# pletzer/nemoflux

Hardware: AMD Instinct MI355X
Metric: edge-flux integrals/sec (higher is better)
Workload: dtype f64; 1 GPU; C4 ORCA12-like 3600x1800x75x12 in total (strong: 900 (t,z) slabs cut 1 way), psi=(1+10*z)*(t+1)*arctan2(y, x+180)/(2*pi), README singular transect + 64 node-snapped transects; nx=3600, ny=1800, nz=75, nt_global=12, target_segments=2229, weight_entries=15468144, parallelism=(t,z)-slab sharding x1, 1 all-reduce, resident_outputs=integratedVelocity [4][ncell] + |eU|,|eV| every step

## Files before the change

nemoflux_amd/csrc/nf_capi_field.hip:

```cpp
#include "nf_capi.h"

using namespace nf;

static int g_batch_steps = 1;
static long g_batch_cellsteps = 32l << 20;
static int g_partial_full = 0;
static int g_use_graph = 1;
static int g_inner_signed = 1;
static int g_k3_pairs = 1;
static int g_inner_interleaved = -1;
static int g_class_window = 32;
static int g_joint_window = 32;
static int g_joint_skip = 1;
static long g_knob_version = 0;

namespace nf {
int field_tuning_set(const char *name, int value)
{
    ++g_knob_version;
    if (!strcmp(name, "batch_steps")) {
        g_batch_steps = value;
        return NF_OK;
    }
    if (!strcmp(name, "batch_cellsteps_m")) {
        if (!(value >= 0 && value <= 2047)) return -1;
        g_batch_cellsteps = (long)value << 20;
        return NF_OK;
    }
    if (!strcmp(name, "partial_step_planes")) {
        g_partial_full = value != 0;
        return NF_OK;
    }
    if (!strcmp(name, "graph")) {
        g_use_graph = value != 0;
        return NF_OK;
    }
    if (!strcmp(name, "pass_inner_signed")) {
        g_inner_signed = value != 0;
        return NF_OK;
    }
    if (!strcmp(name, "pass_k3_pairs")) {
        g_k3_pairs = value != 0;
        return NF_OK;
    }
    if (!strcmp(name, "pass_inner_interleaved")) {
        if (!(value >= -1 && value <= 1)) return -1;
        g_inner_interleaved = value;
        return NF_OK;
    }
    if (!strcmp(name, "class_window")) {
        if (!(value >= 1 && value <= kClassWindowMax)) return -1;
        g_class_window = value;
        return NF_OK;
    }
    if (!strcmp(name, "joint_window")) {
        if (!(value >= 1 && value <= kClassWindowMax)) return -1;
        g_joint_window = value;
        return NF_OK;
    }
    if (!strcmp(name, "joint_skip")) {
        if (!(value == 0 || value == 1)) return -1;
        g_joint_skip = value;
        return NF_OK;
    }
    if (!strcmp(name, "area_chunk")) return area_chunk_set(value);
    if (!strcmp(name, "gross_chunk")) return gross_chunk_set(value);
    if (!strcmp(name, "crossing_chunk")) return crossing_chunk_set(value);
    return -1;
}
}

struct Series {
    const void *p[2] = {nullptr, nullptr};
    long nt = 0;
    int dtype = NF_F64, on_device = 1;
    double fill = std::numeric_limits<double>::quiet_NaN();
    double fill2 = std::numeric_limits<double>::quiet_NaN();
    DevArray<char> stage[2];
};

// ... 352 lines not shown
               std::string(what) + ": this form does not take per-cell thicknesses yet and a cell thickness is set; "
                                   "nf_field_set_cell_thickness(NULL) clears it");
    return NF_OK;
}

static FluxArgs flux_args(const StepInput &in)
{
    return FluxArgs{in.u, in.v, in.dtype, in.ncell, in.ny, in.nx, in.z0, in.z1, in.thickness, in.arcE, in.arcN, in.fill,
                    in.fill2, in.scale, in.sverdrup};
}

static int field_integral(nf_field *f, const double *planes, double *scratch, double *rows, int nsteps = 1,
                          long data_stride = 0, long row_stride = 0)
{
    const Transects tr = field_transects(f);
    return launch_integral(f->ws, planes, f->ncell, 2, f->nx, tr.tr_offsets_dev, tr.ntransect, scratch, rows, f->stream, nsteps,
                           data_stride, row_stride);
}

template <typename Step>
static int field_sync(nf_field *f, size_t n, double *host, Step step)
{
    NF_TRY(f->row.reserve(n > 0 ? n : 1));
    NF_TRY(step(f->row.get()));
    if (host && n > 0) NF_HIP(hipMemcpyAsync(host, f->row.get(), sizeof(double) * n, hipMemcpyDeviceToHost, f->stream));
    NF_HIP(hipStreamSynchronize(f->stream));
    return NF_OK;
}

struct StepForm {
    bool inner = false;
    double *pair_buf = nullptr;
    bool interleaved = false;
};

static int field_step_async(nf_field *f, long t, double *row_dev, StepForm form = {})
{
    const int rowlen = field_row_length(f);
    const bool reduce = row_dev && rowlen > 0 && !form.pair_buf;
    NF_TRY(field_ready(f, "compute", reduce));
    NF_REQUIRE(t >= 0 && t < f->uv.nt, NF_ERR_ARG, "compute: time index out of range");
    const Levels lv = field_levels(f, t);
    if (lv.z1 <= lv.z0) {
        if (row_dev && rowlen > 0) NF_HIP(hipMemsetAsync(row_dev, 0, sizeof(double) * rowlen, f->stream));
        return NF_OK;
    }
    StepInput in;
    NF_TRY(field_step_input(f, t, lv, &in));
    CellThick ct;
    NF_TRY(field_cell_thick(f, t, lv, &ct));
    FluxArgs a = flux_args(in);
    a.iV = f->geo.iV.get();
    if (form.pair_buf) a.iV = form.interleaved ? form.pair_buf : form.pair_buf - f->ncell;
    a.absU = f->geo.abs.get();
    a.absV = f->geo.abs.get() + f->ncell;
    a.maxbits = f->geo.maxbits.get();
    const bool partial = (lv.z0 > 0 || lv.z1 < (int)f->nz) && !g_partial_full;
    a.signed_only = (f->compact || partial || form.inner) && (ct.e3u || flux_supports_signed_only(a));
    NF_REQUIRE(!form.pair_buf || a.signed_only, NF_ERR_STATE, "compute: a step into a pair buffer must be signed-only");
    NF_REQUIRE(!form.interleaved || (form.pair_buf && !ct.e3u && !partial && flux_supports_interleaved(a)), NF_ERR_STATE,
               "compute: the interleaved form is a whole step of a pair on K1's two-field kernel");
    a.interleaved = form.interleaved;
    if (!form.pair_buf) f->derived_stale = a.signed_only != 0;
    NF_TRY(field_launch_flux(f, a, ct.e3u ? &ct : nullptr));
    if (reduce) {
        NF_TRY(field_integral(f, f->geo.iV.get(), f->scratch.get(), row_dev));
        NF_TRY(field_timed_k3_end(f));
    }
    return NF_OK;
}

static int field_raw_step_begin(nf_field *f, const char *what, long t, int tracer, double *rows_dev, size_t nrows, Levels *lv)
{
    const std::string w(what);
    NF_REQUIRE(t >= 0 && t < f->uv.nt, NF_ERR_ARG, w + ": time index out of range");
    if (tracer) NF_TRY(field_matches_uv(f, f->tau.dtype, f->tau.nt, w, "tracer"));
    if (tracer == 2 && f->sig.p[0])
        NF_TRY(field_matches_uv(f, f->sig.dtype, f->sig.nt, w, "class tracer"));
    const size_t rowlen = field_row_length(f);
    *lv = rowlen > 0 ? field_levels(f, t) : Levels{};
    if (rowlen > 0 && lv->z1 <= lv->z0) NF_HIP(hipMemsetAsync(rows_dev, 0, sizeof(double) * rowlen * nrows, f->stream));
    return NF_OK;
}

static int field_tracer_input(nf_field *f, Series &s, long t, Levels lv, TracerIn *in)
{
    NF_TRY(field_stage(f, s, 0, t, lv, &in->tau));
    in->fill = s.fill;
    in->fill2 = s.fill2;
    in->ref = &s == &f->tau ? f->tau_ref : 0.0;
    in->wrap_x = f->tau_wrap;
    return NF_OK;
}

static int field_profile_async(nf_field *f, long t, double *prof_dev, bool tracer = false)
// ... 297 lines not shown
    a.edges = f->class_edges.dev.get();
    a.nedges = nedges;
    a.window = window;
    a.tr = field_transects(f);
    a.scratch = f->class_scratch.get();
    a.scratch_len = f->class_scratch.size();
    a.rows = rows_dev;
    a.nz = (int)f->nz;
    return launch_gross_class_remap(a, f->stream);
}

static int field_class_area_async(nf_field *f, long t, double *rows_dev)
{
    const int nedges = (int)f->class_edges.host.size();
    const size_t nrows = 2 * ((size_t)nedges + 2);
    Levels lv;
    NF_TRY(field_raw_step_begin(f, "compute_class_area", t, 2, rows_dev, nrows, &lv));
    if (lv.z1 <= lv.z0) return NF_OK;
    NF_TRY(f->class_edges.upload((size_t)kMaxClassEdges, f->stream));
    ClassAreaArgs a;
    NF_TRY(field_joint_buffers(f, "compute_class_area", kClassAreaEntryBytes, lv, nrows, &a));
    NF_TRY(field_step_input(f, t, lv, &a.in));
    NF_TRY(field_tracer_input(f, f->tau, t, lv, &a.carry));
    a.cls = a.carry;
    if (f->sig.p[0]) NF_TRY(field_tracer_input(f, f->sig, t, lv, &a.cls));
    NF_TRY(field_cell_thick(f, t, lv, &a.th));
    a.edges = f->class_edges.dev.get();
    a.nedges = nedges;
    a.tr = field_transects(f);
    a.rows = rows_dev;
    return launch_class_area(a, f->stream);
}

static int field_pair_async(nf_field *f, long t, double *rows_dev, bool last, bool last_pair, bool interleaved)
{
    const int rowlen = field_row_length(f);
    StepForm first, second;
    first.inner = true;
    first.pair_buf = f->geo.pair[0].get();
    first.interleaved = interleaved;
    second.inner = g_inner_signed && !last;
    if (interleaved && second.inner && !last_pair) {
        second.pair_buf = f->geo.pair[1].get();
        second.interleaved = true;
    }
    NF_TRY(field_step_async(f, t, nullptr, first));
    NF_TRY(field_step_async(f, t + 1, nullptr, second));
    const double *uvB = second.pair_buf ? second.pair_buf : f->geo.iV.get() + f->ncell;
    NF_TRY(launch_integral_pair(field_transects(f), first.pair_buf, uvB, f->ncell, f->nx, f->scratch.get(),
                                rows_dev + (size_t)t * rowlen, rowlen, f->stream, first.interleaved, second.interleaved));
    NF_TRY(field_timed_k3_end(f));
    return NF_OK;
}

static long batch_cell_steps() { return g_batch_cellsteps; }

static bool field_can_batch(const nf_field *f)
{
    return g_batch_steps && !f->e3.p[0] && f->uv.on_device && f->uv.nt >= 2 && f->uv.nt < 65536 &&
           f->uv.nt * f->ncell <= batch_cell_steps() && f->ncell <= (1l << 20) && f->weights_built;
}

static bool field_pass_pairs(const nf_field *f)
{
    if (!g_k3_pairs || integral_uses_edges() || !f->geo.pair[0].get() || !f->weights_built) return false;
    const size_t step_bytes = (size_t)f->nz * f->ncell * elem_size(f->uv.dtype);
    FluxArgs a{};
    a.u = f->uv.on_device ? f->uv.p[0] : nullptr;
    a.v = f->uv.on_device ? f->uv.p[1] : nullptr;
    a.dtype = f->uv.dtype;
    a.ncell = f->ncell;
    return flux_supports_signed_only(a) && (!f->uv.on_device || step_bytes % 16 == 0);
}

static bool field_pass_interleaved(const nf_field *f)
{
    const bool on = g_inner_interleaved < 0 ? f->uv.dtype == NF_F64 : g_inner_interleaved != 0;
    if (!on || f->compact || f->e3.p[0]) return false;
    FluxArgs a{};
    a.u = f->uv.on_device ? f->uv.p[0] : nullptr;
    a.v = f->uv.on_device ? f->uv.p[1] : nullptr;
    a.dtype = f->uv.dtype;
    a.ncell = f->ncell;
    return flux_supports_interleaved(a);
}

static int field_prepare_pass(nf_field *f)
{
    if (!g_k3_pairs || integral_uses_edges() || !f->geo.iV.get()) return NF_OK;
    const PassSteps p = field_pass_steps(f);
    if (p.wb - p.wa < 2) return NF_OK;
    if (!f->geo.pair[0].get()) NF_TRY(f->geo.pair[0].alloc((size_t)f->ncell * 2));
    if (!f->geo.pair[1].get() && p.wb - p.wa >= 4 && field_pass_interleaved(f)) NF_TRY(f->geo.pair[1].alloc((size_t)f->ncell * 2));
    return NF_OK;
}

static int field_zero_unowned_rows(nf_field *f, double *rows_dev)
{
    const int rowlen = field_row_length(f);
    const PassSteps p = field_pass_steps(f);
    if (rowlen <= 0) return NF_OK;
    if (p.ta > 0) NF_HIP(hipMemsetAsync(rows_dev, 0, sizeof(double) * rowlen * (size_t)p.ta, f->stream));
    if (p.tb < f->uv.nt)
        NF_HIP(hipMemsetAsync(rows_dev + (size_t)p.tb * rowlen, 0, sizeof(double) * rowlen * (size_t)(f->uv.nt - p.tb),
                              f->stream));
    return NF_OK;
}

static int field_all_steps_direct(nf_field *f, double *rows_dev, bool zero_rows = true)
{
    const int rowlen = field_row_length(f);
    const PassSteps p = field_pass_steps(f);
    if (zero_rows) NF_TRY(field_zero_unowned_rows(f, rows_dev));
    const bool pairs = field_pass_pairs(f) && rowlen > 0;
    const long pa = pairs ? p.wa + (p.wb - p.wa) % 2 : p.wb;
    const bool interleaved = pairs && field_pass_interleaved(f) && (p.wb - pa < 4 || f->geo.pair[1].get());
    for (long t = p.ta; t < p.tb;) {
        const bool last = t + 1 == p.tb;
        if (t >= pa && t + 1 < p.wb) {
            NF_TRY(field_pair_async(f, t, rows_dev, t + 2 == p.tb, t + 2 == p.wb, interleaved));
            t += 2;
        } else {
            StepForm form;
            form.inner = g_inner_signed && !last;
            NF_TRY(field_step_async(f, t, rows_dev + (size_t)t * rowlen, form));
            t += 1;
        }
    }
    return NF_OK;
}

static int field_all_steps_batched(nf_field *f, double *rows_dev)
{
    const int rowlen = field_row_length(f);
    const size_t n = (size_t)f->ncell;
    nf_field::Geometry &g = f->geo;
    if (g.batch_steps != f->uv.nt) {
        NF_TRY(g.iVb.alloc(n * 4 * f->uv.nt));
        NF_TRY(g.absb.alloc(n * 2 * f->uv.nt));
        NF_TRY(g.zr.alloc((size_t)2 * f->uv.nt));
        NF_HIP(hipMemsetAsync(g.iVb.get(), 0, sizeof(double) * n * 4 * f->uv.nt, f->stream));
        g.batch_steps = f->uv.nt;
        g.batch_version = -1;
    }
    if (g.batch_version != f->version) {
        NF_TRY(g.scratchb.alloc((size_t)std::max(f->ws.nrec, f->ws.nent) * f->uv.nt));
        std::vector<int> zr((size_t)2 * f->uv.nt);
        for (long t = 0; t < f->uv.nt; ++t) {
            const Levels lv = field_levels(f, t);
            zr[2 * t] = lv.z0;
            zr[2 * t + 1] = lv.z1;
        }
        NF_HIP(hipMemcpy(g.zr.get(), zr.data(), sizeof(int) * zr.size(), hipMemcpyHostToDevice));
// ... 227 lines not shown
    for (size_t p = 0; p < f->polylines.size(); ++p) {
        polyline_segments(f->polylines[p].data(), (int)(f->polylines[p].size() / 3), f->poly_cc[p], segs, cc);
        f->tr_off.push_back((int)cc.size());
    }
    f->weights_built = false;
    f->prof_scratch.reset();
    f->tprof_scratch.reset();
    f->area_scratch.reset();
    f->gross_scratch.reset();
    f->crossings.reset();
    f->class_scratch.reset();
    f->joint_table.reset();
    f->joint_flags.reset();
    f->joint_scratch.reset();
    const int bw = build_weights(f->geo.xy.get(), f->ncell, segs.data(), cc.data(), (int)cc.size(), periodX, &f->ws, f->stream,
                                 f->skip_unsupported, f->overlap_warn, nullptr, f->nx);
    if (bw != NF_OK) {
        for (size_t q = 0; q < f->ws.coverage.size(); ++q)
            if ((long)q == (long)f->ws.over_seg) {
                size_t p = 0;
                while (p + 2 < f->tr_off.size() && (size_t)f->tr_off[p + 1] <= q) ++p;
                char buf[320];
                snprintf(buf, sizeof buf,
                         "nf_field_build_weights: transect %zu, target segment %zu is covered %.9g times by the cells of the "
                         "grid: cells overlap along it (a cell wrapped across the date line with periodX = 0, or duplicated "
                         "/ folded cells that are not identical), so part of the line would be counted twice",
                         p, q - (size_t)f->tr_off[p], f->ws.coverage[q]);
                set_error(buf);
                break;
            }
        return bw;
    }
    if (integral_uses_edges()) NF_TRY(fold_weights(&f->ws, f->ncell, f->nx, f->stream));
    NF_TRY(f->tr_off_dev.alloc(f->tr_off.size()));
    NF_TRY(f->scratch.alloc((size_t)2 * std::max(f->ws.nrec, f->ws.nent)));
    NF_HIP(hipMemcpy(f->tr_off_dev.get(), f->tr_off.data(), sizeof(int) * f->tr_off.size(), hipMemcpyHostToDevice));
    f->weights_built = true;
    ++f->version;
    return NF_OK;
}
NF_API_CATCH

int nf_field_num_transects(nf_field **self, int *n)
try {
    NF_REQUIRE(self && *self && n, NF_ERR_ARG, "nf_field_num_transects: null argument");
    *n = (int)(*self)->polylines.size();
    return NF_OK;
}
NF_API_CATCH
int nf_field_num_segments(nf_field **self, int *nseg_total)
try {
    NF_REQUIRE(self && *self && nseg_total, NF_ERR_ARG, "nf_field_num_segments: null argument");
    NF_REQUIRE((*self)->weights_built, NF_ERR_STATE, "nf_field_num_segments: build_weights first");
    *nseg_total = (*self)->ws.nseg;
    return NF_OK;
}
NF_API_CATCH
int nf_field_segment_offsets(nf_field **self, int *offsets)
try {
    NF_REQUIRE(self && *self && offsets, NF_ERR_ARG, "nf_field_segment_offsets: null argument");
    NF_REQUIRE((*self)->weights_built, NF_ERR_STATE, "nf_field_segment_offsets: build_weights first");
    memcpy(offsets, (*self)->tr_off.data(), sizeof(int) * (*self)->tr_off.size());
    return NF_OK;
}
NF_API_CATCH
int nf_field_num_weights(nf_field **self, size_t *n)
// ... 933 lines not shown
```

nemoflux_amd/csrc/nf_common.h:

```cpp
#pragma once
#include <hip/hip_runtime.h>
#include <cstdint>
#include <cstdio>
#include <string>
#include <cmath>
#include <initializer_list>
#include <mutex>
#include <vector>

#include "../../include/nemoflux_amd.h"

namespace nf {

constexpr int kWave = 64;
constexpr int kBlock = 256;
constexpr int kXcds = 8;
constexpr double kDeg2Rad = 3.14159265358979323846 / 180.0;
constexpr double kEarthRadiusSv = 6371000.0;

void set_error(const std::string &msg);
int hip_fail(hipError_t e, const char *what, const char *file, int line);

#define NF_HIP(call)                                                   \
    do {                                                               \
// ... 78 lines not shown
    double m = 1.0;
    for (double c : {seg4[0], seg4[1], seg4[0] + seg4[2], seg4[1] + seg4[3]}) m = std::fabs(c) > m ? std::fabs(c) : m;
    return (cov - 1.0) * len > kCoverLenTol * m;
}

int launch_geometry(const void *blon, const void *blat, int dtype, long ncell, double *xy, double *arc4,
                    double *arcE, double *arcN, unsigned long long *box_keys, hipStream_t s);
int launch_corner_table_from_points(const double *points, long ncell, double *xy, hipStream_t s);
int launch_points_from_corner_table(const double *xy, long ncell, double *points, hipStream_t s);
double box_key_to_double(unsigned long long k);

struct StepBatch {
    int nsteps = 0;
    long in_stride = 0;
    const int *zr = nullptr;
};

struct FluxArgs {
    const void *u, *v;
    int dtype;
    long ncell, ny, nx;
    int z0, z1;
    const double *thickness;
    const double *arcE, *arcN;
    double fill;
    double fill2 = __builtin_nan("");
    double scale;
    int sverdrup;
    double *iV, *absU, *absV;
    unsigned long long *maxbits;
    StepBatch batch;
    int signed_only = 0;
    int interleaved = 0;
    hipEvent_t mid_event = nullptr;
    bool *mid_recorded = nullptr;
};
int launch_flux(const FluxArgs &a, hipStream_t s);
bool flux_supports_signed_only(const FluxArgs &a);
bool flux_supports_interleaved(const FluxArgs &a);
int launch_expand_planes(double *iV, double *absUV, long ncell, long ny, long nx, hipStream_t s);
int tuning_set(const char *name, int value);
long tuning_version();
int launch_planes_to_aos(const double *planes, long ncell, double *aos, hipStream_t s);

template <typename T>
class DevArray {
public:
    DevArray() = default;
    DevArray(const DevArray &) = delete;
    DevArray &operator=(const DevArray &) = delete;
    DevArray(DevArray &&o) noexcept : p_(o.p_), n_(o.n_) { o.p_ = nullptr, o.n_ = 0; }
    DevArray &operator=(DevArray &&o) noexcept
    {
        if (this != &o) {
            reset();
            p_ = o.p_, n_ = o.n_;
            o.p_ = nullptr, o.n_ = 0;
        }
        return *this;
    }
    ~DevArray() { reset(); }
    int alloc(size_t n)
    {
        reset();
        void *q = nullptr;
        NF_HIP(hipMalloc(&q, n ? sizeof(T) * n : (sizeof(T) > 16 ? sizeof(T) : 16)));
        p_ = static_cast<T *>(q);
        n_ = n ? n : 1;
        return NF_OK;
    }
    int reserve(size_t n, bool *grown = nullptr)
    {
// ... 3 lines not shown
    }
    void reset()
    {
        if (p_) (void)hipFree(p_);
        p_ = nullptr, n_ = 0;
    }
    T *get() const { return p_; }
    size_t size() const { return n_; }

private:
    T *p_ = nullptr;
    size_t n_ = 0;
};

struct WeightSet {
    long nrec = 0;
    DevArray<int> cell;
    DevArray<double> w4;
    DevArray<int> seg;
    DevArray<double> tab;
    int nseg = 0;
    DevArray<int> seg_start;
    std::vector<double> coverage;
    int over_seg = -1;
    long dropped = 0;
    struct EdgeEntry {
        int elem;
        int seg;
        double w;
    };
    long nent = 0;
    DevArray<EdgeEntry> ent;
    DevArray<int> ent_start;
    long entries() const { return 4 * nrec; }
    void release() { *this = WeightSet(); }
};
int fold_weights(WeightSet *ws, long ncell, long nx, hipStream_t s);
int weights_to_host(const WeightSet &ws, int64_t *cell_edge, double *weight, int *seg);
struct Box4;
struct LocatorBoxes {
    std::vector<DevArray<Box4>> level;
    std::vector<long> count;
    const double *xy = nullptr;
    long ncell = 0;
    double period = -1.0;
    std::mutex mtx;
    void release();
};
int build_weights(const double *xy, long ncell, const double *segs_host, const int *seg_cc_host, int nseg,
                  double periodX, WeightSet *out, hipStream_t s, int skip_unsupported = 0, int overlap_warn = 0,
                  LocatorBoxes *boxes = nullptr, long row_length = 0);
void weights_trim_scratch();

struct Transects {
    const WeightSet *ws = nullptr;
    const int *tr_offsets_dev = nullptr;
    int ntransect = 0;
    long row_length() const { return ws->nseg + ntransect; }
};

void integral_use_edges(int on);
int integral_uses_edges();
int launch_integral(const WeightSet &ws, const double *data, long ncell, int planes, long nx,
                    const int *tr_offsets_dev, int ntransect, double *scratch, double *row, hipStream_t s,
                    int nsteps = 1, long data_stride = 0, long row_stride = 0, const int *rec_cells = nullptr);
int launch_integral_pair(const Transects &tr, const double *uvA, const double *uvB, long ncell, long nx, double *scratch,
                         double *row, long row_stride, hipStream_t s, bool a_interleaved = false, bool b_interleaved = false);

struct StepInput {
// ... 299 lines not shown
```

nemoflux_amd/csrc/nf_flux.hip:

```cpp
#include <cstring>

#include "nf_common.h"

namespace nf {

template <typename T, int VEC> struct vec_t;
typedef double dvec2 __attribute__((ext_vector_type(2)));
typedef float fvec4 __attribute__((ext_vector_type(4)));
template <> struct vec_t<double, 2> { using type = dvec2; };
template <> struct vec_t<float, 4> { using type = fvec4; };
template <> struct vec_t<double, 1> { using type = double; };
template <> struct vec_t<float, 1> { using type = float; };

template <typename T, int VEC> struct Lanes {
    T x[VEC];
};

template <typename T, int VEC, bool NT>
__device__ inline Lanes<T, VEC> load_cells(const T *p)
{
    using V = typename vec_t<T, VEC>::type;
    Lanes<T, VEC> r;
    V v = NT ? __builtin_nontemporal_load(reinterpret_cast<const V *>(p)) : *reinterpret_cast<const V *>(p);
    __builtin_memcpy(&r, &v, sizeof(V));
// ... 50 lines not shown
        if (j0 + 1 < ny) store1<NTS>(p0 + c0 + nx, eV[0]);
        store1<NTS>(p3 + ((i0 + 1 < nx) ? c0 + 1 : c0 + 1 - nx), eU[0]);
    } else {
#pragma unroll
        for (int k = 0; k < VEC; k += 2) {
            store2<NTS>(p1 + c0 + k, eU[k], eU[k + 1], true);
            store2<NTS>(p2 + c0 + k, eV[k], eV[k + 1], true);
            store2<NTS>(aU + c0 + k, fabs(eU[k]), fabs(eU[k + 1]), true);
            store2<NTS>(aV + c0 + k, fabs(eV[k]), fabs(eV[k + 1]), true);
        }
        if (i0 + VEC <= nx) {
            if (j0 + 1 < ny) {
                const bool al = (nx & 1u) == 0;
#pragma unroll
                for (int k = 0; k < VEC; k += 2) store2<NTS>(p0 + c0 + nx + k, eV[k], eV[k + 1], al);
            }
#pragma unroll
            for (int k = 0; k < VEC; ++k) store1<NTS>(p3 + ((i0 + k + 1 < nx) ? c0 + k + 1 : c0 + k + 1 - nx), eU[k]);
        } else {
#pragma unroll
            for (int k = 0; k < VEC; ++k) {
                const long c = c0 + k;
                const unsigned j = (unsigned)(c / nx);
                const unsigned i = (unsigned)(c - (long)j * nx);
                if (j + 1 < ny) store1<NTS>(p0 + c + nx, eV[k]);
                store1<NTS>(p3 + ((i + 1 < nx) ? c + 1 : c + 1 - nx), eU[k]);
            }
        }
    }
}

constexpr int kFormSignedOnly = 16;
constexpr int kFormInterleaved = 32;
constexpr int kFormNestedLoads = 128;
constexpr int kFormTwoFills = 256;
#ifdef NF_TUNING_BUILD
constexpr int kDiagNoStores = 1, kDiagNoFix = 2, kDiagNoMax = 4, kDiagNoArc = 8, kDiagPlainStores = 64;
#else
constexpr int kDiagNoStores = 0, kDiagNoFix = 0, kDiagNoMax = 0, kDiagNoArc = 0, kDiagPlainStores = 0;
#endif

template <typename T, int VEC, int UZ, bool NT, int BLOCK, int CH, int FORM = 0>
__global__ __launch_bounds__(BLOCK) void k_flux(const T *__restrict__ u, const T *__restrict__ v, long ncell,
                                                unsigned ny, unsigned nx, int z0, int z1,
                                                const double *__restrict__ thickness,
                                                const double *__restrict__ arcE, const double *__restrict__ arcN,
                                                T fill, double scale, int sverdrup, double *__restrict__ iV,
                                                double *__restrict__ absUV, unsigned long long *maxbits,
                                                unsigned ntiles, int xcd_map, StepBatch sb, T fill2)
{
#ifndef NF_TUNING_BUILD
    static_assert((FORM & ~(kFormSignedOnly | kFormInterleaved | kFormNestedLoads | kFormTwoFills)) == 0, "diagnostic forms exist only in tuning builds");
#endif
    const unsigned tile = xcd_map ? xcd_tile(blockIdx.x, gridDim.x) : blockIdx.x;
    if (sb.zr) {
        const long tb = blockIdx.y;
        u += tb * sb.in_stride;
        v += tb * sb.in_stride;
        iV += tb * 4 * ncell;
        absUV += tb * 2 * ncell;
        z0 = sb.zr[2 * tb];
        z1 = sb.zr[2 * tb + 1];
    }
    double tmax = 0.0;
    if (tile < ntiles) {
        const long base = (long)tile * BLOCK * VEC * CH + (long)threadIdx.x * VEC;
        constexpr long kChunk = (long)BLOCK * VEC;
        bool on[CH];
        double accU[CH][VEC], accV[CH][VEC];
#pragma unroll
        for (int q = 0; q < CH; ++q) {
            on[q] = base + q * kChunk < ncell;
#pragma unroll
            for (int k = 0; k < VEC; ++k) accU[q][k] = accV[q][k] = 0.0;
        }
        const T *pu = u + (long)z0 * ncell + base;
        const T *pv = v + (long)z0 * ncell + base;
        for (int z = z0; z < z1; z += UZ) {
            const int nlev = z1 - z < UZ ? z1 - z : UZ;
            Lanes<T, VEC> lu[UZ][CH], lv[UZ][CH];
            if (CH == 1 && !(FORM & kFormNestedLoads)) {
#pragma unroll
                for (int k = 0; k < 2 * UZ; ++k) {
                    const int r = k / 2;
                    if (r < nlev && on[0]) {
                        if ((k & 1) == 0) lu[r][0] = load_cells<T, VEC, NT>(pu + (long)r * ncell);
                        else lv[r][0] = load_cells<T, VEC, NT>(pv + (long)r * ncell);
                    }
                }
            } else {
#pragma unroll
                for (int r = 0; r < UZ; ++r)
                    if (r < nlev) {
#pragma unroll
                        for (int q = 0; q < CH; ++q)
                            if (on[q]) {
                                lu[r][q] = load_cells<T, VEC, NT>(pu + (long)r * ncell + q * kChunk);
                                lv[r][q] = load_cells<T, VEC, NT>(pv + (long)r * ncell + q * kChunk);
                            }
                    }
            }
#pragma unroll
            for (int r = 0; r < UZ; ++r)
                if (r < nlev) {
                    const double th = thickness[z + r];
#pragma unroll
                    for (int q = 0; q < CH; ++q)
                        if (on[q]) {
#pragma unroll
                            for (int k = 0; k < VEC; ++k) {
                                if (FORM & kFormTwoFills) {
                                    accU[q][k] = fma(th, fixed2<T>(lu[r][q].x[k], fill, fill2), accU[q][k]);
                                    accV[q][k] = fma(th, fixed2<T>(lv[r][q].x[k], fill, fill2), accV[q][k]);
                                } else {
                                    accU[q][k] = fma(th, (FORM & kDiagNoFix) ? (double)lu[r][q].x[k] : fixed<T>(lu[r][q].x[k], fill), accU[q][k]);
                                    accV[q][k] = fma(th, (FORM & kDiagNoFix) ? (double)lv[r][q].x[k] : fixed<T>(lv[r][q].x[k], fill), accV[q][k]);
                                }
                            }
                        }
                }
            pu += (long)UZ * ncell;
            pv += (long)UZ * ncell;
        }
#pragma unroll
        for (int q = 0; q < CH; ++q)
            if (on[q]) {
                const long c0 = base + q * kChunk;
                double eU[VEC], eV[VEC];
#pragma unroll
                for (int k = 0; k < VEC; ++k) {
                    eU[k] = +accU[q][k] * ((FORM & kDiagNoArc) ? 1.5 : arcE[c0 + k]);
                    eV[k] = -accV[q][k] * ((FORM & kDiagNoArc) ? 1.5 : arcN[c0 + k]);
                    if (sverdrup) {
                        eU[k] *= scale;
                        eV[k] *= scale;
                    }
                    tmax = fmax(tmax, fmax(fabs(eU[k]), fabs(eV[k])));
                }
                if (FORM & kFormInterleaved) {
#pragma unroll
                    for (int k = 0; k < VEC; ++k) store2<true>(iV + 2 * (c0 + k), eU[k], eV[k], true);
                } else if (FORM & kFormSignedOnly) {
#pragma unroll
                    for (int k = 0; k < VEC; k += 2) {
                        store2<true>(iV + ncell + c0 + k, eU[k], eU[k + 1], true);
                        store2<true>(iV + 2 * ncell + c0 + k, eV[k], eV[k + 1], true);
                    }
                } else if (!(FORM & kDiagNoStores)) store_cells<VEC, !(FORM & kDiagPlainStores)>(c0, eU, eV, ncell, ny, nx, iV, absUV);
            }
    }
    for (int o = 32; o > 0; o >>= 1) tmax = fmax(tmax, __shfl_xor(tmax, o, kWave));
    if ((threadIdx.x & (kWave - 1)) == 0 && tmax > 0.0 && !(FORM & kDiagNoMax)) {
        unsigned long long b;
        __builtin_memcpy(&b, &tmax, 8);
        if (b > __hip_atomic_load(maxbits, __ATOMIC_RELAXED, __HIP_MEMORY_SCOPE_AGENT)) atomicMax(maxbits, b);
    }
}

template <typename T, int VEC, int UZ, bool SIGNED_ONLY, bool TWO_FILLS, bool WSHIFT = false>
__global__ __launch_bounds__(256) void k_flux_field(const T *__restrict__ u, const T *__restrict__ v, long ncell,
                                                    unsigned ny, unsigned nx, int z0, int z1,
                                                    const double *__restrict__ thickness,
                                                    const double *__restrict__ arcE, const double *__restrict__ arcN,
                                                    T fill, double scale, int sverdrup, double *__restrict__ iV,
                                                    double *__restrict__ absUV, unsigned long long *maxbits,
                                                    unsigned ntiles, int xcd_map, StepBatch sb, T fill2)
{
    const unsigned tile = xcd_map ? xcd_tile(blockIdx.x, gridDim.x) : blockIdx.x;
    const bool is_v = blockIdx.z != 0;
    if (sb.zr) {
        const long tb = blockIdx.y;
        u += tb * sb.in_stride;
        v += tb * sb.in_stride;
        iV += tb * 4 * ncell;
// ... 193 lines not shown
    NF_HIP(hipGetLastError());
    return NF_OK;
}

template <typename T, int VEC>
static int launch_flux_field(const FluxArgs &a, hipStream_t s)
{
    constexpr int kLevels = sizeof(T) == 8 ? 10 : 16;
    const bool two = (T)a.fill2 == (T)a.fill2 && !((T)a.fill2 == (T)a.fill);
    if (a.signed_only)
        return two ? launch_flux_field_t<T, VEC, kLevels, true, true>(a, s) : launch_flux_field_t<T, VEC, kLevels, true, false>(a, s);
    if (g_west_shift && VEC > 1)
        return two ? launch_flux_field_t<T, VEC, kLevels, false, true, true>(a, s) : launch_flux_field_t<T, VEC, kLevels, false, false, true>(a, s);
    return two ? launch_flux_field_t<T, VEC, kLevels, false, true>(a, s) : launch_flux_field_t<T, VEC, kLevels, false, false>(a, s);
}

static bool takes_field_form(const FluxArgs &a, int vec)
{
    if ((a.batch.zr ? 0 : g_variant) != 0) return false;
    const long waves = (a.ncell / vec + kWave - 1) / kWave;
    return g_field_split < 0 ? (!a.batch.zr && waves < kFieldSplitWaves) : g_field_split != 0;
}

template <typename T, int VEC>
static int launch_flux_v(const FluxArgs &a, hipStream_t s)
{
    const int variant = a.batch.zr ? 0 : g_variant;
    const bool two = (T)a.fill2 == (T)a.fill2 && !((T)a.fill2 == (T)a.fill);
    if (a.interleaved) {
        if constexpr (VEC > 1) {
            NF_REQUIRE(a.signed_only && !a.batch.zr && !takes_field_form(a, VEC), NF_ERR_STATE,
                       "flux: the interleaved form is a signed-only step of the two-field kernel");
            constexpr int kLevels = sizeof(T) == 8 ? 10 : 8;
            if (two) return launch_flux_t<T, VEC, kLevels, true, 256, 1, kFormSignedOnly | kFormInterleaved | kFormTwoFills>(a, s);
            return launch_flux_t<T, VEC, kLevels, true, 256, 1, kFormSignedOnly | kFormInterleaved>(a, s);
        }
        NF_REQUIRE(false, NF_ERR_STATE, "flux: the interleaved form needs 16-byte aligned fields and an even cell count");
    }
    if (takes_field_form(a, VEC)) return launch_flux_field<T, VEC>(a, s);
    if (a.signed_only) {
        NF_REQUIRE(VEC > 1 && !a.batch.zr, NF_ERR_STATE, "flux: the compact mode needs 16-byte aligned fields, an even cell count and one step per launch");
        if (two) return launch_flux_t<T, VEC, (sizeof(T) == 8 ? 10 : 8), true, 256, 1, kFormSignedOnly | kFormTwoFills>(a, s);
        return launch_flux_t<T, VEC, (sizeof(T) == 8 ? 10 : 8), true, 256, 1, kFormSignedOnly>(a, s);
    }
    if (VEC == 1) {
        if (two) return launch_flux_t<T, VEC, 8, true, 256, 1, kFormTwoFills>(a, s);
        return launch_flux_t<T, VEC, 8, true, 256, 1>(a, s);
    }
    if (two) {
        constexpr int kLevels = sizeof(T) == 8 ? 10 : 8;
        if (a.batch.zr || sizeof(T) == 8) return launch_flux_t<T, VEC, kLevels, true, 256, 1, kFormTwoFills>(a, s);
        const int rc = launch_flux_t<T, VEC, kLevels, true, 256, 1, kFormSignedOnly | kFormTwoFills>(a, s);
        if (rc != NF_OK) return rc;
        if (a.mid_event) {
            NF_HIP(hipEventRecord(a.mid_event, s));
            if (a.mid_recorded) *a.mid_recorded = true;
        }
        return launch_expand_planes(a.iV, a.absU, a.ncell, a.ny, a.nx, s);
    }
    switch (variant) {
#ifdef NF_TUNING_BUILD
        case 3: return launch_flux_t<T, VEC, 4, true, 256, 1>(a, s);
        case 4: return launch_flux_t<T, VEC, 4, true, 256, 2>(a, s);
        case 11: return launch_flux_t<T, VEC, 10, false, 256, 1>(a, s);
        case 12: return launch_flux_t<T, VEC, 8, true, 256, 1>(a, s);
        case 14: return launch_flux_t<T, VEC, 16, true, 256, 1>(a, s);
// ... 5 lines not shown
        case 45: return launch_flux_ww<T, VEC, 2, 2>(a, s);
        case 6: {
            const int rc = launch_flux_t<T, VEC, (sizeof(T) == 8 ? 10 : 8), true, 256, 1, kFormSignedOnly | kFormNestedLoads>(a, s);
            return rc != NF_OK ? rc : launch_expand_planes(a.iV, a.absU, a.ncell, a.ny, a.nx, s);
        }
#endif
        case 5:
        default: {
            constexpr int kLevels = sizeof(T) == 8 ? 10 : 8;
            const bool fused = a.batch.zr || ((sizeof(T) == 8) != (variant == 5));
            if (fused) return launch_flux_t<T, VEC, kLevels, true, 256, 1>(a, s);
            const int rc = launch_flux_t<T, VEC, kLevels, true, 256, 1, kFormSignedOnly>(a, s);
            if (rc != NF_OK) return rc;
            if (a.mid_event) {
                NF_HIP(hipEventRecord(a.mid_event, s));
                if (a.mid_recorded) *a.mid_recorded = true;
            }
            return launch_expand_planes(a.iV, a.absU, a.ncell, a.ny, a.nx, s);
        }
    }
}

bool flux_supports_signed_only(const FluxArgs &a)
{
    const bool al16 = ((uintptr_t)a.u % 16 == 0) && ((uintptr_t)a.v % 16 == 0);
    return al16 && !a.batch.zr && a.ncell % (a.dtype == NF_F32 ? 4 : 2) == 0;
}

bool flux_supports_interleaved(const FluxArgs &a)
{
    return flux_supports_signed_only(a) && !takes_field_form(a, a.dtype == NF_F32 ? 4 : 2);
}

int launch_flux(const FluxArgs &a, hipStream_t s)
{
    NF_REQUIRE(a.ncell > 0 && a.ncell == a.ny * a.nx && a.ncell < (1l << 31), NF_ERR_ARG, "flux: bad grid sizes");
    NF_REQUIRE(a.batch.zr || (a.z1 > a.z0 && a.z0 >= 0), NF_ERR_ARG, "flux: empty z range");
    NF_REQUIRE(!a.batch.zr || (a.batch.nsteps > 0 && a.batch.nsteps < 65536), NF_ERR_ARG, "flux: bad step batch");
    NF_REQUIRE(a.absV == a.absU + a.ncell, NF_ERR_ARG, "flux: abs planes must be contiguous");
    const bool al16 = ((uintptr_t)a.u % 16 == 0) && ((uintptr_t)a.v % 16 == 0);
    if (a.dtype == NF_F64) {
        if (al16 && a.ncell % 2 == 0) return launch_flux_v<double, 2>(a, s);
        return launch_flux_v<double, 1>(a, s);
    } else if (a.dtype == NF_F32) {
        if (al16 && a.ncell % 4 == 0) return launch_flux_v<float, 4>(a, s);
        return launch_flux_v<float, 1>(a, s);
    }
    NF_REQUIRE(false, NF_ERR_ARG, "flux: dtype must be NF_F64 or NF_F32");
}

__global__ __launch_bounds__(kBlock) void k_planes_to_aos(const double *__restrict__ planes, long ncell,
                                                          double *__restrict__ aos)
{
    long c = (long)blockIdx.x * kBlock + threadIdx.x;
    if (c < ncell) {
        double2 *o = reinterpret_cast<double2 *>(aos + 4 * c);
        o[0] = make_double2(planes[c], planes[ncell + c]);
        o[1] = make_double2(planes[2 * ncell + c], planes[3 * ncell + c]);
    }
}
int launch_planes_to_aos(const double *planes, long ncell, double *aos, hipStream_t s)
{
    hipLaunchKernelGGL(k_planes_to_aos, dim3((unsigned)((ncell + kBlock - 1) / kBlock)), dim3(kBlock), 0, s,
                       planes, ncell, aos);
    NF_HIP(hipGetLastError());
    return NF_OK;
// ... 4 lines not shown
```

nemoflux_amd/csrc/nf_integral.hip:

```cpp
#include <type_traits>

#include "nf_common.h"

namespace nf {

typedef double dvec2 __attribute__((ext_vector_type(2)));

struct Record {
    long c;
    dvec2 wa, wb;
};
__device__ inline Record load_record(const int *__restrict__ cell, const double *__restrict__ w4, long k)
{
    const dvec2 *pw = reinterpret_cast<const dvec2 *>(w4 + 4 * k);
    return Record{__builtin_nontemporal_load(cell + k), __builtin_nontemporal_load(pw), __builtin_nontemporal_load(pw + 1)};
}
__device__ inline int load_key(const int *__restrict__ seg, long k) { return __builtin_nontemporal_load(seg + k); }

struct Neighbours {
    unsigned j, i;
    bool south;
    long cs, cw;
};
__device__ inline Neighbours neighbours(long c, unsigned nx)
// ... 413 lines not shown

int launch_integral(const WeightSet &ws, const double *data, long ncell, int planes, long nx,
                    const int *tr_offsets_dev, int ntransect, double *scratch, double *row, hipStream_t s, int nsteps,
                    long data_stride, long row_stride, const int *rec_cells)
{
    const Transects tr{&ws, tr_offsets_dev, ntransect};
    const unsigned ny = (unsigned)(nsteps > 1 ? nsteps : 1);
    const bool edges = planes == 2 && ws.ent_start.get() && g_use_edges;
    if (edges && ws.nent > 0)
        hipLaunchKernelGGL(k_gather_edges, dim3((unsigned)((ws.nent + kBlock - 1) / kBlock), ny), dim3(kBlock), 0, s,
                           ws.ent.get(), ws.nent, data, ncell, scratch, data_stride);
    if (!edges && ws.nrec > 0)
        hipLaunchKernelGGL(k_gather_segscan, record_grid(ws, ny), dim3(kBlock), 0, s,
                           rec_cells ? rec_cells : ws.cell.get(), ws.w4.get(), ws.seg.get(), ws.nrec, data, ncell, planes,
                           (unsigned)(nx > 0 ? nx : 1), scratch, data_stride);
    launch_finalize(tr, edges ? ws.ent_start.get() : ws.seg_start.get(), edges ? ws.nent : ws.nrec, scratch, row, row_stride,
                    ny, s);
    NF_HIP(hipGetLastError());
    return NF_OK;
}

int launch_integral_pair(const Transects &tr, const double *uvA, const double *uvB, long ncell, long nx, double *scratch,
                         double *row, long row_stride, hipStream_t s, bool a_interleaved, bool b_interleaved)
{
    const WeightSet &ws = *tr.ws;
    NF_REQUIRE(a_interleaved || !b_interleaved, NF_ERR_ARG, "integral: operand B is interleaved only when A is");
    if (ws.nrec > 0) {
        auto *kernel = b_interleaved ? k_gather_segscan_pair<true, true>
                                     : (a_interleaved ? k_gather_segscan_pair<true, false> : k_gather_segscan_pair<false, false>);
        hipLaunchKernelGGL(kernel, record_grid(ws), dim3(kBlock), 0, s, ws.cell.get(), ws.w4.get(), ws.seg.get(), ws.nrec,
                           uvA, uvB, ncell, (unsigned)(nx > 0 ? nx : 1), scratch);
    }
    launch_finalize(tr, ws.seg_start.get(), ws.nrec, scratch, row, row_stride, 2, s);
    NF_HIP(hipGetLastError());
    return NF_OK;
}

static int check_raw_step(const char *what, const StepInput &in, const Transects &tr, size_t scratch_len, size_t per_record)
{
    const std::string w(what);
    NF_REQUIRE(tr.ws && in.ncell > 0 && in.nx > 0 && in.ncell % in.nx == 0 && in.ncell < (1l << 31), NF_ERR_ARG,
               w + ": bad grid sizes");
    NF_REQUIRE(in.z0 >= 0 && in.z1 >= in.z0 && tr.ntransect >= 0, NF_ERR_ARG, w + ": bad arguments");
    NF_REQUIRE(scratch_len >= (size_t)tr.ws->nrec * per_record, NF_ERR_ARG, w + ": scratch too small");
    return NF_OK;
}

template <typename T, int LZ, typename... TI>
__global__ __launch_bounds__(kBlock) void k_profile_segscan(const int *__restrict__ cell, const double *__restrict__ w4,
                                                            const int *__restrict__ seg, long n, const T *__restrict__ u,
                                                            const T *__restrict__ v, long ncell, unsigned nx, int z0,
                                                            int nlev, const double *__restrict__ thickness,
                                                            const double *__restrict__ arcE,
                                                            const double *__restrict__ arcN, T fill, T fill2, int two,
                                                            double scale, int sverdrup, double *__restrict__ runsum,
                                                            TI... tracer)
{
    constexpr bool TR = (std::is_same<TI, TauIn<T>>::value || ...);
    constexpr bool CT = (std::is_same<TI, ThickIn<T>>::value || ...);
    const TauIn<T> ti = tau_in<T>(tracer...);
    const ThickIn<T> ct = thick_arg<T>(tracer...);
    const long k = (long)blockIdx.x * kBlock + threadIdx.x;
    double val[LZ];
#pragma unroll
    for (int l = 0; l < LZ; ++l) val[l] = 0.0;
    int key = -1;
// ... 1577 lines not shown
```

Before: 382.7 billion integrals/s.

## Mask interleaved pair-buffer stores to cells the transect weights read

Result: no change. 384.0 billion integrals/s, median of 6 (+0.3%).

```diff
diff --git a/nemoflux_amd/csrc/nf_capi_field.hip b/nemoflux_amd/csrc/nf_capi_field.hip
--- a/nemoflux_amd/csrc/nf_capi_field.hip
+++ b/nemoflux_amd/csrc/nf_capi_field.hip
@@ -9,6 +9,8 @@
 static int g_inner_signed = 1;
 static int g_k3_pairs = 1;
 static int g_inner_interleaved = -1;
+static int g_inner_sparse = -1;
+static int g_pair_poison = 0;
 static int g_class_window = 32;
 static int g_joint_window = 32;
 static int g_joint_skip = 1;
@@ -46,6 +48,16 @@
     if (!strcmp(name, "pass_inner_interleaved")) {
         if (!(value >= -1 && value <= 1)) return -1;
         g_inner_interleaved = value;
+        return NF_OK;
+    }
+    if (!strcmp(name, "pass_inner_sparse")) {
+        if (!(value >= -1 && value <= 1)) return -1;
+        g_inner_sparse = value;
+        return NF_OK;
+    }
+    if (!strcmp(name, "pass_pair_poison")) {
+        if (!(value == 0 || value == 1)) return -1;
+        g_pair_poison = value;
         return NF_OK;
     }
     if (!strcmp(name, "class_window")) {
@@ -464,6 +476,7 @@
     bool inner = false;
     double *pair_buf = nullptr;
     bool interleaved = false;
+    bool sparse = false;
 };
 
 static int field_step_async(nf_field *f, long t, double *row_dev, StepForm form = {})
@@ -493,6 +506,12 @@
     NF_REQUIRE(!form.interleaved || (form.pair_buf && !ct.e3u && !partial && flux_supports_interleaved(a)), NF_ERR_STATE,
                "compute: the interleaved form is a whole step of a pair on K1's two-field kernel");
     a.interleaved = form.interleaved;
+    if (form.sparse) {
+        NF_REQUIRE(form.interleaved && f->weights_built && f->ws.need.get() && flux_supports_sparse(a), NF_ERR_STATE,
+                   "compute: the sparse form is an interleaved float64 step under the need-mask of the built weights");
+        a.need = f->ws.need.get();
+        a.need_words = f->ws.need.size();
+    }
     if (!form.pair_buf) f->derived_stale = a.signed_only != 0;
     NF_TRY(field_launch_flux(f, a, ct.e3u ? &ct : nullptr));
     if (reduce) {
@@ -856,17 +875,19 @@
     return launch_class_area(a, f->stream);
 }
 
-static int field_pair_async(nf_field *f, long t, double *rows_dev, bool last, bool last_pair, bool interleaved)
+static int field_pair_async(nf_field *f, long t, double *rows_dev, bool last, bool last_pair, bool interleaved, bool sparse)
 {
     const int rowlen = field_row_length(f);
     StepForm first, second;
     first.inner = true;
     first.pair_buf = f->geo.pair[0].get();
     first.interleaved = interleaved;
+    first.sparse = interleaved && sparse;
     second.inner = g_inner_signed && !last;
     if (interleaved && second.inner && !last_pair) {
         second.pair_buf = f->geo.pair[1].get();
         second.interleaved = true;
+        second.sparse = sparse;
     }
     NF_TRY(field_step_async(f, t, nullptr, first));
     NF_TRY(field_step_async(f, t + 1, nullptr, second));
@@ -909,13 +930,22 @@
     return flux_supports_interleaved(a);
 }
 
+static bool field_pass_sparse(const nf_field *f)
+{
+    const bool on = g_inner_sparse < 0 ? f->uv.dtype == NF_F64 : g_inner_sparse != 0;
+    return on && f->uv.dtype == NF_F64 && f->weights_built && f->ws.need.get() && field_pass_interleaved(f);
+}
+
 static int field_prepare_pass(nf_field *f)
 {
     if (!g_k3_pairs || integral_uses_edges() || !f->geo.iV.get()) return NF_OK;
     const PassSteps p = field_pass_steps(f);
     if (p.wb - p.wa < 2) return NF_OK;
-    if (!f->geo.pair[0].get()) NF_TRY(f->geo.pair[0].alloc((size_t)f->ncell * 2));
-    if (!f->geo.pair[1].get() && p.wb - p.wa >= 4 && field_pass_interleaved(f)) NF_TRY(f->geo.pair[1].alloc((size_t)f->ncell * 2));
+    for (int b = 0; b < 2; ++b) {
+        if (f->geo.pair[b].get() || (b == 1 && !(p.wb - p.wa >= 4 && field_pass_interleaved(f)))) continue;
+        NF_TRY(f->geo.pair[b].alloc((size_t)f->ncell * 2));
+        if (g_pair_poison) NF_HIP(hipMemsetAsync(f->geo.pair[b].get(), 0xff, sizeof(double) * 2 * (size_t)f->ncell, f->stream));
+    }
     return NF_OK;
 }
 
@@ -939,10 +969,11 @@
     const bool pairs = field_pass_pairs(f) && rowlen > 0;
     const long pa = pairs ? p.wa + (p.wb - p.wa) % 2 : p.wb;
     const bool interleaved = pairs && field_pass_interleaved(f) && (p.wb - pa < 4 || f->geo.pair[1].get());
+    const bool sparse = interleaved && field_pass_sparse(f);
     for (long t = p.ta; t < p.tb;) {
         const bool last = t + 1 == p.tb;
         if (t >= pa && t + 1 < p.wb) {
-            NF_TRY(field_pair_async(f, t, rows_dev, t + 2 == p.tb, t + 2 == p.wb, interleaved));
+            NF_TRY(field_pair_async(f, t, rows_dev, t + 2 == p.tb, t + 2 == p.wb, interleaved, sparse));
             t += 2;
         } else {
             StepForm form;
@@ -1236,6 +1267,7 @@
         return bw;
     }
     if (integral_uses_edges()) NF_TRY(fold_weights(&f->ws, f->ncell, f->nx, f->stream));
+    NF_TRY(build_need_mask(&f->ws, f->ncell, f->nx, f->stream));
     NF_TRY(f->tr_off_dev.alloc(f->tr_off.size()));
     NF_TRY(f->scratch.alloc((size_t)2 * std::max(f->ws.nrec, f->ws.nent)));
     NF_HIP(hipMemcpy(f->tr_off_dev.get(), f->tr_off.data(), sizeof(int) * f->tr_off.size(), hipMemcpyHostToDevice));
diff --git a/nemoflux_amd/csrc/nf_common.h b/nemoflux_amd/csrc/nf_common.h
--- a/nemoflux_amd/csrc/nf_common.h
+++ b/nemoflux_amd/csrc/nf_common.h
@@ -134,12 +134,21 @@
     StepBatch batch;
     int signed_only = 0;
     int interleaved = 0;
+    const unsigned *need = nullptr;
+    size_t need_words = 0;
     hipEvent_t mid_event = nullptr;
     bool *mid_recorded = nullptr;
 };
 int launch_flux(const FluxArgs &a, hipStream_t s);
 bool flux_supports_signed_only(const FluxArgs &a);
 bool flux_supports_interleaved(const FluxArgs &a);
+bool flux_supports_sparse(const FluxArgs &a);
+#ifndef NF_NEED_GRANULE
+#define NF_NEED_GRANULE 4
+#endif
+constexpr int kNeedGranule = NF_NEED_GRANULE;
+static_assert(kNeedGranule == 2 || kNeedGranule == 4 || kNeedGranule == 8, "a need-mask bit stands for 2, 4 or 8 cells");
+inline size_t need_mask_words(long ncell) { return (size_t)((ncell + 511) / 512) * (512 / kNeedGranule / 32); }
 int launch_expand_planes(double *iV, double *absUV, long ncell, long ny, long nx, hipStream_t s);
 int tuning_set(const char *name, int value);
 long tuning_version();
@@ -209,9 +218,11 @@
     long nent = 0;
     DevArray<EdgeEntry> ent;
     DevArray<int> ent_start;
+    DevArray<unsigned> need;
     long entries() const { return 4 * nrec; }
     void release() { *this = WeightSet(); }
 };
+int build_need_mask(WeightSet *ws, long ncell, long nx, hipStream_t s);
 int fold_weights(WeightSet *ws, long ncell, long nx, hipStream_t s);
 int weights_to_host(const WeightSet &ws, int64_t *cell_edge, double *weight, int *seg);
 struct Box4;
diff --git a/nemoflux_amd/csrc/nf_flux.hip b/nemoflux_amd/csrc/nf_flux.hip
--- a/nemoflux_amd/csrc/nf_flux.hip
+++ b/nemoflux_amd/csrc/nf_flux.hip
@@ -106,6 +106,7 @@
 
 constexpr int kFormSignedOnly = 16;
 constexpr int kFormInterleaved = 32;
+constexpr int kFormSparse = 512;
 constexpr int kFormNestedLoads = 128;
 constexpr int kFormTwoFills = 256;
 #ifdef NF_TUNING_BUILD
@@ -124,8 +125,10 @@
                                                 unsigned ntiles, int xcd_map, StepBatch sb, T fill2)
 {
 #ifndef NF_TUNING_BUILD
-    static_assert((FORM & ~(kFormSignedOnly | kFormInterleaved | kFormNestedLoads | kFormTwoFills)) == 0, "diagnostic forms exist only in tuning builds");
+    static_assert((FORM & ~(kFormSignedOnly | kFormInterleaved | kFormSparse | kFormNestedLoads | kFormTwoFills)) == 0, "diagnostic forms exist only in tuning builds");
 #endif
+    static_assert(!(FORM & kFormSparse) || ((FORM & kFormInterleaved) && sizeof(T) == 8 && VEC == 2 && CH == 1),
+                  "the sparse form is the float64 interleaved form with its stores masked");
     const unsigned tile = xcd_map ? xcd_tile(blockIdx.x, gridDim.x) : blockIdx.x;
     if (sb.zr) {
         const long tb = blockIdx.y;
@@ -147,6 +150,15 @@
             on[q] = base + q * kChunk < ncell;
 #pragma unroll
             for (int k = 0; k < VEC; ++k) accU[q][k] = accV[q][k] = 0.0;
+        }
+        bool need = true;
+        if (FORM & kFormSparse) {
+            const unsigned *mask = reinterpret_cast<const unsigned *>(absUV);
+            constexpr int kWaveBits = kWave * VEC / kNeedGranule;
+            const unsigned wbit = __builtin_amdgcn_readfirstlane((tile * BLOCK + (threadIdx.x & ~(unsigned)(kWave - 1))) * VEC / kNeedGranule);
+            const unsigned lbit = (threadIdx.x & (kWave - 1)) * VEC / kNeedGranule;
+            if (kWaveBits == 64) need = (*reinterpret_cast<const unsigned long long *>(mask + wbit / 32) >> lbit) & 1;
+            else need = (mask[wbit / 32] >> (wbit % 32 + lbit)) & 1;
         }
         const T *pu = u + (long)z0 * ncell + base;
         const T *pv = v + (long)z0 * ncell + base;
@@ -212,8 +224,10 @@
                     tmax = fmax(tmax, fmax(fabs(eU[k]), fabs(eV[k])));
                 }
                 if (FORM & kFormInterleaved) {
-#pragma unroll
-                    for (int k = 0; k < VEC; ++k) store2<true>(iV + 2 * (c0 + k), eU[k], eV[k], true);
+                    if (!(FORM & kFormSparse) || need) {
+#pragma unroll
+                        for (int k = 0; k < VEC; ++k) store2<true>(iV + 2 * (c0 + k), eU[k], eV[k], true);
+                    }
                 } else if (FORM & kFormSignedOnly) {
 #pragma unroll
                     for (int k = 0; k < VEC; k += 2) {
@@ -473,6 +487,16 @@
             NF_REQUIRE(a.signed_only && !a.batch.zr && !takes_field_form(a, VEC), NF_ERR_STATE,
                        "flux: the interleaved form is a signed-only step of the two-field kernel");
             constexpr int kLevels = sizeof(T) == 8 ? 10 : 8;
+            if constexpr (sizeof(T) == 8) {
+                if (a.need) {
+                    NF_REQUIRE(a.need_words >= need_mask_words(a.ncell), NF_ERR_ARG, "flux: the need-mask is too short for the grid");
+                    FluxArgs b = a;
+                    b.absU = reinterpret_cast<double *>(const_cast<unsigned *>(a.need));
+                    if (two) return launch_flux_t<T, VEC, kLevels, true, 256, 1, kFormSignedOnly | kFormInterleaved | kFormSparse | kFormTwoFills>(b, s);
+                    return launch_flux_t<T, VEC, kLevels, true, 256, 1, kFormSignedOnly | kFormInterleaved | kFormSparse>(b, s);
+                }
+            }
+            NF_REQUIRE(!a.need, NF_ERR_STATE, "flux: the sparse form is a float64 form");
             if (two) return launch_flux_t<T, VEC, kLevels, true, 256, 1, kFormSignedOnly | kFormInterleaved | kFormTwoFills>(a, s);
             return launch_flux_t<T, VEC, kLevels, true, 256, 1, kFormSignedOnly | kFormInterleaved>(a, s);
         }
@@ -544,6 +568,8 @@
     return flux_supports_signed_only(a) && !takes_field_form(a, a.dtype == NF_F32 ? 4 : 2);
 }
 
+bool flux_supports_sparse(const FluxArgs &a) { return a.dtype == NF_F64 && flux_supports_interleaved(a); }
+
 int launch_flux(const FluxArgs &a, hipStream_t s)
 {
     NF_REQUIRE(a.ncell > 0 && a.ncell == a.ny * a.nx && a.ncell < (1l << 31), NF_ERR_ARG, "flux: bad grid sizes");
diff --git a/nemoflux_amd/csrc/nf_integral.hip b/nemoflux_amd/csrc/nf_integral.hip
--- a/nemoflux_amd/csrc/nf_integral.hip
+++ b/nemoflux_amd/csrc/nf_integral.hip
@@ -469,6 +469,32 @@
                            uvA, uvB, ncell, (unsigned)(nx > 0 ? nx : 1), scratch);
     }
     launch_finalize(tr, ws.seg_start.get(), ws.nrec, scratch, row, row_stride, 2, s);
+    NF_HIP(hipGetLastError());
+    return NF_OK;
+}
+
+__global__ __launch_bounds__(kBlock) void k_need_mask(const int *__restrict__ cell, long n, unsigned nx,
+                                                      unsigned *__restrict__ need)
+{
+    const long k = (long)blockIdx.x * kBlock + threadIdx.x;
+    if (k >= n) return;
+    const long c = cell[k];
+    const Neighbours nb = neighbours(c, nx);
+    auto set = [&](long x) { atomicOr(need + x / (32 * kNeedGranule), 1u << (unsigned)(x / kNeedGranule % 32)); };
+    set(c);
+    set(nb.cw);
+    if (nb.south) set(nb.cs);
+}
+
+int build_need_mask(WeightSet *ws, long ncell, long nx, hipStream_t s)
+{
+    NF_REQUIRE(ncell > 0 && nx > 0 && ncell % nx == 0 && ncell < (1l << 31), NF_ERR_ARG, "need-mask: bad grid sizes");
+    const size_t words = need_mask_words(ncell);
+    NF_TRY(ws->need.alloc(words));
+    NF_HIP(hipMemsetAsync(ws->need.get(), 0, sizeof(unsigned) * words, s));
+    if (ws->nrec > 0)
+        hipLaunchKernelGGL(k_need_mask, record_grid(*ws), dim3(kBlock), 0, s, ws->cell.get(), ws->nrec, (unsigned)nx,
+                           ws->need.get());
     NF_HIP(hipGetLastError());
     return NF_OK;
 }
```
